# wwood/CoverM

Measured on AMD Instinct MI355X. Metric: aligned reads/s through coverm contig (mean trimmed_mean covered_fraction variance), higher is better.
Workload: dtype i32 depth / u64 sums / f32 estimators

## Files before the change

### coverm_amd/csrc/covermhip.hip

```cpp
#include "pileup_kernels.hip.h"
#include "prep_lean.hip.h"
#include "genome_kernels.hip.h"
#include "sep_kernels.hip.h"
#include "ingest_kernels.hip.h"
#include "group_kernels.hip.h"
#include "sam_kernels.hip.h"

#include <algorithm>
#include <atomic>
#include <cstddef>
#include <chrono>
#include <cstdio>
#include <dlfcn.h>
#include <functional>
#include <sched.h>
#include <cstdlib>
#include <cstring>
#include <map>
#include <mutex>
#include <string>
#include <future>
#include <thread>
#include <vector>

// ... 911 lines not shown
    if (s) s->merged_valid = false;
    cov_summary local;
    cov_status st = finish_store(s, stats, (s && s->spill.active && !summary) ? &local : summary);
    if (st == COV_OK && s->spill.active) st = merge_spilled(s, stats, summary ? summary : &local);
    return st;
}

cov_status cov_finish_genomes(cov_session *s, cov_summary *summary) {
    covr::Range rr("cov_finish_genomes");
    if (!s) return COV_ERR_INVALID_ARG;
    s->merged_valid = false;
    if (s->spill.active) { s->err = "cov_finish_genomes: part of the sample's contigs left the bounded record store: cov_finish, and aggregate on the host"; return COV_ERR_STATE; }
    s->lean_finish = true;
    const cov_status st = finish_store(s, nullptr, summary);
    s->lean_finish = false;
    return st;
}

static cov_status finish_once(cov_session *s, cov_contig_stats *stats, cov_summary *summary, bool &again) {
    again = false;
    if (!s || (!stats && s->n_targets && !s->lean_finish)) return COV_ERR_INVALID_ARG;
    const bool lean = s->lean_finish;
    s->depth_all_valid = false;
    HIPCHK(hipSetDevice(s->cfg.device));
    timing_events(s);
    hipStream_t st = s->stream;
    const u32 nT = s->n_targets;
    const u32 R = (u32)s->store.n_records;
    const bool want_hist = s->cfg.want & COV_WANT_HIST, want_id = s->cfg.want & COV_WANT_IDENTITY;
    for (int k = 0; k < COV_K_COUNT; k++) { s->k_launches[k] = 0; s->k_ms[k] = 0.f; }
    bool compacted = false;
    s->est_valid = false; s->gen_valid = false;
    s->ev_fresh = -1;

    HIPCHK(s->d_runs.reserve(std::max<size_t>(1, R), st));
    const uint64_t ncig_all = s->adopted ? s->adopted_ncig : s->store.n_cigar;
    const bool long_cigars = R && ncig_all / R >= 16;
    const int prep_kernel = s->prep_kernel;
    const int prep_passes = long_cigars ? 1 : 2 * PREP_PASSES, prep_b = 1;
    const u32 prep_chunk = (u32)(256 * prep_b * prep_passes);
    const u32 prep_grid = (R + prep_chunk - 1) / prep_chunk;
    HIPCHK(s->d_part.reserve((size_t)prep_grid + 2, st));
    if (want_id) {
        if (!(s->cfg.want & COV_WANT_IDENTITY_PRIMARY_ONLY)) HIPCHK(s->d_ident.reserve(std::max<size_t>(1, R), st));
        if (!(s->cfg.want & COV_WANT_IDENTITY_NONSUPP_ONLY)) HIPCHK(s->d_identp.reserve(std::max<size_t>(1, R), st));
        HIPCHK(s->d_idch.reserve((size_t)R / ID_CH + 2, st));
    }
    if (want_hist) HIPCHK(s->d_arena.reserve((size_t)R + nT + 1, st));

    TileIdx ti{};
    ti.tile_first = s->d_tile_first.p; ti.tcnt = s->d_tcnt.p; ti.fov = s->d_fov.p; ti.shift = s->tile_shift; ti.n_tiles = s->n_tiles;
    CxIdx cx{};
    {
        const uint64_t ncig_now = s->adopted ? s->adopted_ncig : s->store.n_cigar;
        HIPCHK(s->d_cx_list.reserve((size_t)(ncig_now / CX_MIN_OPS) + 64, st));
        cx.list = s->d_cx_list.p; cx.list_cap = (u32)std::min<uint64_t>(ncig_now / CX_MIN_OPS + 64, 0xffffffffull);
        cx.cnt = s->d_cx_cnt.p; cx.cur = s->d_cx_cur.p; cx.cscan = s->d_cx_scan.p; cx.ctop = s->d_cx_top.p;
        cx.runs = s->d_cx_runs.p; cx.runs_cap = s->d_cx_runs.cap;
    }
    const Records r = records_of(s);
    const uint8_t *mask = s->have_mask ? s->d_mask.p : nullptr;
    FilterCfg f{};
    f.include_improper_pairs = s->cfg.include_improper_pairs; f.include_supplementary = s->cfg.include_supplementary;
    f.include_secondary = s->cfg.include_secondary; f.filter_single = s->cfg.filter_single;
    f.min_mapq = s->cfg.min_mapq; f.min_aligned_length = s->cfg.min_aligned_length;
    f.min_percent_identity = s->cfg.min_percent_identity; f.min_aligned_percent = s->cfg.min_aligned_percent;
    double *idp = (want_id && !(s->cfg.want & COV_WANT_IDENTITY_NONSUPP_ONLY)) ? s->d_identp.p : nullptr;
    double *idn = (want_id && !(s->cfg.want & COV_WANT_IDENTITY_PRIMARY_ONLY)) ? s->d_ident.p : nullptr;
    HIPCHK(s->d_prep_args.reserve(1, st));
    HIPCHK(s->d_gen_list.reserve((size_t)R / 64 + 2, st));
    PrepArgs pa{};
    {
        PrepHot &ph = pa.hot;
        ph.tid = r.tid; ph.pos = r.pos; ph.flag = r.flag; ph.nmk = r.nm_kind; ph.nm = r.nm; ph.coff = r.cigar_off; ph.cigar = r.cigar; ph.mapq = r.mapq; ph.lseq = r.l_seq;
        ph.runs = s->d_runs.p; ph.tcnt = ti.tcnt; ph.fov = ti.fov; ph.identp = idp; ph.identn = idn;
        ph.n = r.n; ph.cigar_end = r.cigar_end; ph.n_targets = nT; ph.shift = ti.shift; ph.steps = (u32)prep_chunk / 256u;
        ph.gate_mask = 0x4u | (f.include_secondary ? 0u : 0x100u) | (f.include_supplementary ? 0u : 0x800u) | (f.include_improper_pairs ? 0u : 0x2u);
        ph.p1_mask = 0x4u | (f.include_secondary ? 0u : 0x100u) | (f.include_supplementary ? 0u : 0x800u);
        ph.min_mapq = f.min_mapq; ph.min_aligned_length = f.min_aligned_length; ph.min_percent_identity = f.min_percent_identity; ph.min_aligned_percent = f.min_aligned_percent;
        PrepCold &pc = pa.cold;
        pc.ctg = s->d_ctg.p; pc.g = s->d_glob.p; pc.part = s->d_part.p; pc.cx_list = cx.list; pc.mask = mask; pc.tlen = s->d_tlen.p; pc.tile_first = s->d_tile_first.p;
        pc.cx_list_cap = cx.list_cap; pc.gen_list = s->d_gen_list.p;
    }
    hipLaunchKernelGGL(k_init, dim3((std::max(std::max(nT, COUNTER_SLOTS * 8), s->n_tiles) + 255) / 256), dim3(256), 0, st, s->d_ctg.p,
                       nT, s->d_glob.p, ti, cx, s->d_prep_args.p, pa);
    HIPCHK(hipGetLastError());

    if (R) {
        time_begin(s, COV_K_PREP);
        const u32 n_steps = (R + 63u) / 64u;
        const bool gen_all = prep_kernel != 7 && (uint64_t)R < (uint64_t)nT * 128u;
        s->last_gen_all = gen_all;
        const u32 gen_grid = gen_all ? std::min<u32>((u32)s->n_cus * 64u, (n_steps + 3u) / 4u) : std::min<u32>((u32)s->n_cus * 8u, (n_steps + 3u) / 4u);
#define COV_LAUNCH_PREP(ID, FI, MA)                                                                                                       \
        do {                                                                                                                              \
            if (prep_kernel == 7)                                                                                                         \
                hipLaunchKernelGGL((k_prep7s<ID, FI, MA>), dim3(prep_grid), dim3(256), 0, st, r, s->d_tlen.p, nT, mask, f, s->d_ctg.p,   \
                                   s->d_glob.p, s->d_runs.p, idp, idn, s->d_part.p, ti, prep_passes, prep_b, cx.list, cx.list_cap);      \
            else if (gen_all)                                                                                                             \
                hipLaunchKernelGGL((k_prep_generic<ID, FI, MA>), dim3(gen_grid), dim3(256), 0, st, (const PrepArgs *)s->d_prep_args.p, n_steps); \
            else {                                                                                                                        \
                hipLaunchKernelGGL((k_prep_lean<ID, FI, MA>), dim3(prep_grid), dim3(256), 0, st, pa.hot, (const PrepArgs *)s->d_prep_args.p); \
                hipLaunchKernelGGL((k_prep_generic<ID, FI, MA>), dim3(gen_grid), dim3(256), 0, st, (const PrepArgs *)s->d_prep_args.p, 0u); \
            }                                                                                                                             \
        } while (0)
        {
            const int key = (want_id ? 4 : 0) | (s->cfg.filter_single ? 2 : 0) | (mask != nullptr ? 1 : 0);
            switch (key) {
            case 0: COV_LAUNCH_PREP(false, false, false); break;
            case 1: COV_LAUNCH_PREP(false, false, true); break;
            case 2: COV_LAUNCH_PREP(false, true, false); break;
            case 3: COV_LAUNCH_PREP(false, true, true); break;
            case 4: COV_LAUNCH_PREP(true, false, false); break;
            case 5: COV_LAUNCH_PREP(true, false, true); break;
            case 6: COV_LAUNCH_PREP(true, true, false); break;
            default: COV_LAUNCH_PREP(true, true, true); break;
            }
        }
#undef COV_LAUNCH_PREP
        if (nT) {
            const u32 n_red = gen_all ? 0u : (nT + 3u) / 4u, cx_grid0 = (u32)s->n_cus * 8u;
            hipLaunchKernelGGL(k_post_prep, dim3(n_red + cx_grid0), dim3(256), 0, st, r, s->d_tlen.p, s->d_glob.p, cx, ti, s->d_ctg.p, nT, (const PrepPartial *)s->d_part.p,
                               prep_grid, prep_chunk, n_red);
        }
        time_end(s, COV_K_PREP);
        HIPCHK(hipGetLastError());
        if (want_id && nT) {
            if (!s->side) {
                (void)ingest_prep_wait(s);
                if (s->ing_aux && !s->ing_active) s->side = s->ing_aux;
                else { HIPCHK(hipStreamCreateWithFlags(&s->side, hipStreamNonBlocking)); s->side_owned = true; }
            }
            HIPCHK(hipEventRecord(s->ev_prep_done, st));
            HIPCHK(hipStreamWaitEvent(s->side, s->ev_prep_done, 0));
            (void)hipEventRecord(s->ev[COV_K_IDENTITY][0], s->side);
            if (s->id_mode) {
                const u32 nch = (R + ID_CH - 1) / ID_CH;
                hipLaunchKernelGGL(k_id_approx, dim3(nch), dim3(256), 0, s->side, idp, idn, R, s->d_idch.p);
                hipLaunchKernelGGL(k_id_predict, dim3(nT), dim3(64), 0, s->side, s->d_ctg.p, nT, idp, idn, s->d_idch.p);
                hipLaunchKernelGGL(k_id_exact, dim3(nch), dim3(256), 0, s->side, idp, idn, R, s->d_idch.p);
                hipLaunchKernelGGL(k_id_combine, dim3(nT), dim3(64), 0, s->side, s->d_ctg.p, nT, idp, idn, r.tid, s->d_idch.p);
            } else
                hipLaunchKernelGGL(k_identity, dim3(nT), dim3(64), 0, s->side, s->d_ctg.p, nT, idp, idn, r.tid);
            (void)hipEventRecord(s->ev[COV_K_IDENTITY][1], s->side);
            s->k_launches[COV_K_IDENTITY]++;
            HIPCHK(hipGetLastError());
            HIPCHK(hipEventRecord(s->ev_side_done, s->side));
            s->ev_fresh = -1;
        }
    }
    if (R && s->n_tiles) {
        time_begin(s, COV_K_RANGES);
        const u32 n_blocks = (s->n_tiles + 1023u) / 1024u;
        const u32 cx_grid = (u32)s->n_cus * 8u;
        ScanPair sp{};
        sp.cnt[0] = s->d_tcnt.p; sp.scan[0] = s->d_tscan.p; sp.top[0] = s->d_ttop.p; sp.total[0] = nullptr;
        sp.cnt[1] = s->d_cx_cnt.p; sp.scan[1] = s->d_cx_scan.p; sp.top[1] = s->d_cx_top.p; sp.total[1] = &s->d_glob.p->cx_total;
        hipLaunchKernelGGL(k_tile_scan1, dim3(2u * n_blocks), dim3(1024), 0, st, sp, s->n_tiles, n_blocks);
        hipLaunchKernelGGL(k_tile_scan2, dim3(2), dim3(1024), 0, st, sp, n_blocks);
        hipLaunchKernelGGL((k_cx_expand<true>), dim3(cx_grid), dim3(256), 0, st, r, s->d_tlen.p, s->d_glob.p, cx, ti);
        u32 *slow_list = s->use_fast ? s->d_slow_list.p : nullptr;
        if (want_hist)
            hipLaunchKernelGGL((k_ranges<true>), dim3((s->n_tiles + 255) / 256), dim3(256), 0, st, s->d_tile_contig.p,
                               s->d_tile_start.p, s->n_tiles, s->d_tlen.p, mask, s->d_ctg.p, s->d_desc.p, ti, s->d_tscan.p,
                               s->d_ttop.p, cx, s->d_glob.p, slow_list);
        else
            hipLaunchKernelGGL((k_ranges<false>), dim3((s->n_tiles + 255) / 256), dim3(256), 0, st, s->d_tile_contig.p,
                               s->d_tile_start.p, s->n_tiles, s->d_tlen.p, mask, s->d_ctg.p, s->d_desc.p, ti, s->d_tscan.p,
                               s->d_ttop.p, cx, s->d_glob.p, slow_list);
        time_end(s, COV_K_RANGES);
        HIPCHK(hipGetLastError());
        if (want_hist) {
            time_begin(s, COV_K_HIST);
            const u32 hb = (nT + 1023u) / 1024u;
            HIPCHK(s->d_hist_top.reserve(hb, st));
            hipLaunchKernelGGL((k_hist_sum<0>), dim3(hb), dim3(1024), 0, st, (const DevContig *)s->d_ctg.p, nT, s->d_tlen.p, mask, (u64)s->cfg.contig_end_exclusion, s->d_hist_top.p);
            hipLaunchKernelGGL((k_hist_off<0>), dim3(hb), dim3(1024), 0, st, s->d_ctg.p, nT, s->d_tlen.p, mask, (u64)s->cfg.contig_end_exclusion, (const u64 *)s->d_hist_top.p, s->d_glob.p);
            hipLaunchKernelGGL(k_zero_u32, dim3(2048), dim3(256), 0, st, s->d_arena.p, &s->d_glob.p->hist_cap_total);
            time_end(s, COV_K_HIST);
            HIPCHK(hipGetLastError());
        }
        PileupArgs a = pileup_args(s);
        time_begin(s, COV_K_PILEUP);
        if (want_hist) launch_any_pileup<true, false>(s, a, s->n_tiles);
        else launch_any_pileup<false, false>(s, a, s->n_tiles);
        time_end(s, COV_K_PILEUP);
        HIPCHK(hipGetLastError());
        if (want_hist) {
            compacted = s->est.n == 0 || s->hist_fetch_seen;
            s->hist_prefetched = 0;
            if (compacted) {
                HIPCHK(s->d_chist.reserve((size_t)R + nT + 1, st));
                time_begin(s, COV_K_HIST_COMPACT);
                const u32 hb = (nT + 1023u) / 1024u;
                hipLaunchKernelGGL((k_hist_sum<1>), dim3(hb), dim3(1024), 0, st, (const DevContig *)s->d_ctg.p, nT, s->d_tlen.p, mask, (u64)s->cfg.contig_end_exclusion, s->d_hist_top.p);
                hipLaunchKernelGGL((k_hist_off<1>), dim3(hb), dim3(1024), 0, st, s->d_ctg.p, nT, s->d_tlen.p, mask, (u64)s->cfg.contig_end_exclusion, (const u64 *)s->d_hist_top.p, s->d_glob.p);
                hipLaunchKernelGGL(k_hist_compact, dim3((nT + 3u) / 4u), dim3(256), 0, st, s->d_ctg.p, nT, s->d_tlen.p, (u64)s->cfg.contig_end_exclusion, s->d_arena.p, s->d_chist.p);
                time_end(s, COV_K_HIST_COMPACT);
                HIPCHK(hipGetLastError());
                const u64 guess = s->hist_fetch_seen ? std::min<u64>({s->last_chist_total + s->last_chist_total / 16, (u64)R + nT + 1, (u64)(64u << 20) / 8}) : 0;
                if (guess) {
                    if (guess > s->h_chist_cap) {
                        if (s->h_chist) (void)hipHostFree(s->h_chist);
                        s->h_chist = nullptr; s->h_chist_cap = 0;
                        HIPCHK(hipHostMalloc((void **)&s->h_chist, (size_t)guess * 8, hipHostMallocDefault));
                        s->h_chist_cap = guess;
                    }
                    HIPCHK(hipMemcpyAsync(s->h_chist, s->d_chist.p, (size_t)guess * 8, hipMemcpyDeviceToHost, st));
                    s->hist_prefetched = guess;
                }
            }
            s->hist_fetch_seen = false;
        }
    }
    const size_t block = result_block_bytes(nT), nf = (s->have_mask || s->have_runs) ? 0 : (size_t)nT * s->est.n;
    {
        result_host_take(s);
        const size_t need = lean ? sizeof(DevGlobal) + sizeof(DevContig) : result_host_bytes(s, nT);
        if (need > s->h_res_cap) {
            if (s->h_res) (void)hipHostFree(s->h_res);
            s->h_res = nullptr; s->h_res_cap = 0;
            const size_t cap = need < ((size_t)64 << 20) ? need + need / 2 : need;
            HIPCHK(hipHostMalloc((void **)&s->h_res, cap, hipHostMallocDefault));
            s->h_res_cap = cap;
        }
        s->h_ctg = (DevContig *)(s->h_res + sizeof(DevGlobal));
        s->h_estf = reinterpret_cast<float *>(s->h_res + block);
    }
    if (want_id && R && nT) { HIPCHK(hipStreamWaitEvent(st, s->ev_side_done, 0)); s->ev_fresh = -1; }
    if (nf) {
        time_begin(s, COV_K_ESTIMATE);
        if (s->est_lanes < 0 ? nT >= 65536u : s->est_lanes == 1)
            hipLaunchKernelGGL(k_estimate_lanes, dim3((nT + 255) / 256), dim3(256), 0, st, (const DevContig *)s->d_ctg.p, nT, (const u32 *)s->d_tlen.p, (u64)s->cfg.contig_end_exclusion,
                               (const u32 *)s->d_arena.p, s->est, reinterpret_cast<float *>(s->d_res.p + block));
        else
            hipLaunchKernelGGL(k_estimate, dim3((nT + 3) / 4), dim3(256), 0, st, (const DevContig *)s->d_ctg.p, nT, (const u32 *)s->d_tlen.p, (u64)s->cfg.contig_end_exclusion,
                               (const u32 *)s->d_arena.p, s->est, reinterpret_cast<float *>(s->d_res.p + block));
        time_end(s, COV_K_ESTIMATE);
        HIPCHK(hipGetLastError());
    }
    const bool runs = s->have_runs && s->est.n != 0 && !s->spill.active && !s->in_spill;
    const bool genomes = runs || (s->have_genomes && s->est.n != 0 && !s->spill.active && !s->in_spill);
    if (lean && !genomes) { s->err = "cov_finish_genomes: cov_set_genomes or cov_set_genome_runs, and cov_set_estimators, first, and no spill of the bounded record store (cov_finish then)"; return COV_ERR_STATE; }
    u32 sep_counts[SEP_N_COUNTS] = {0, 0, 0, 0};
    if (runs) {
        const u32 nb = (std::max(nT, 1u) + SEP_TILE - 1u) / SEP_TILE, eb = (s->sep_ent_cap + SEP_TILE - 1u) / SEP_TILE, cap = s->sep_ent_cap;
        time_begin(s, COV_K_SEP);
        hipLaunchKernelGGL(k_sep_obs_top, dim3(nb), dim3(SEP_TILE), 0, st, (const DevContig *)s->d_ctg.p, nT, s->d_stop_last1.p, s->d_stop_first.p);
        hipLaunchKernelGGL(k_sep_flags, dim3(nb), dim3(SEP_TILE), 0, st, (const DevContig *)s->d_ctg.p, nT, (const int32_t *)s->d_sgid.p, (const u32 *)s->d_sblk.p,
                           (const u32 *)s->d_stop_last1.p, (const u32 *)s->d_stop_first.p, s->d_scode.p, s->d_stop_cnt.p);
        hipLaunchKernelGGL(k_sep_compact, dim3(nb), dim3(SEP_TILE), 0, st, nT, (const int32_t *)s->d_sgid.p, (const u32 *)s->d_sblk.p, (const uint8_t *)s->d_scode.p,
                           (const u64 *)s->d_stop_cnt.p, s->d_gtids.p, s->d_sent_pos.p, s->d_sent.p, cap, s->d_scounts.p, s->d_glob.p);
        hipLaunchKernelGGL(k_sep_rows, dim3((std::max(nT, 1u) + 255u) / 256u), dim3(256), 0, st, (const u32 *)s->d_scounts.p, (const u32 *)s->d_sent_pos.p, s->d_grow.p, cap);
        hipLaunchKernelGGL(k_sep_seg_sum, dim3(eb), dim3(SEP_TILE), 0, st, (const u32 *)s->d_scounts.p, (const u32 *)s->d_grow.p, s->d_stop_seg.p);
        hipLaunchKernelGGL(k_sep_seg_write, dim3(eb), dim3(SEP_TILE), 0, st, s->d_scounts.p, (const u32 *)s->d_grow.p, (const u64 *)s->d_stop_seg.p, s->d_gseg_genome.p,
                           s->d_gseg_start.p, s->sep_seg_cap);
        time_end(s, COV_K_SEP);
        HIPCHK(hipGetLastError());
        uint8_t *hc = s->h_gout + s->h_gout_cap - 16;
        HIPCHK(hipMemcpyAsync(hc, s->d_scounts.p, SEP_N_COUNTS * sizeof(u32), hipMemcpyDeviceToHost, st));
        HIPCHK(hipStreamSynchronize(st));
        memcpy(sep_counts, hc, sizeof sep_counts);
        s->ev_fresh = -1;
        s->n_genomes = sep_counts[SEP_N_ENTRIES]; s->n_gseg = sep_counts[SEP_N_SEG];
    }
    if (genomes && s->n_genomes != 0) {
        const u32 nG = s->n_genomes, n_seg = s->n_gseg, sep = runs ? 1u : 0u;
        GenomeTable gt{s->d_grow.p, s->d_gtids.p, s->d_gseg_genome.p, s->d_gseg_start.p, nG, n_seg};
        const u64 excl = s->cfg.contig_end_exclusion;
        const u64 ghist_cap = (u64)R + nT + 1;
        if (want_hist) HIPCHK(s->d_ghist.reserve((size_t)ghist_cap, st));
        time_begin(s, COV_K_GENOME);
        hipLaunchKernelGGL(k_genome_init, dim3((nG + 255u) / 256u), dim3(256), 0, st, s->d_genomes.p, nG);
        if (n_seg) hipLaunchKernelGGL(k_genome_reduce, dim3((n_seg + 3u) / 4u), dim3(256), 0, st, (const DevContig *)s->d_ctg.p, (const u32 *)s->d_tlen.p, excl, gt, s->d_genomes.p, sep);
        if (want_id && !(s->cfg.want & (runs ? COV_WANT_IDENTITY_NONSUPP_ONLY : COV_WANT_IDENTITY_PRIMARY_ONLY)))
            hipLaunchKernelGGL(k_genome_identity, dim3(nG), dim3(64), 0, st, (const DevContig *)s->d_ctg.p, gt, s->d_genomes.p, sep);
        if (want_hist) {
            const u32 gb = (nG + 1023u) / 1024u;
            u64 *total = s->d_ghist_top.p + gb;
            hipLaunchKernelGGL(k_genome_hist_sum, dim3(gb), dim3(1024), 0, st, (const DevGenome *)s->d_genomes.p, nG, s->d_ghist_top.p);
            hipLaunchKernelGGL(k_genome_hist_off, dim3(gb), dim3(1024), 0, st, s->d_genomes.p, nG, (const u64 *)s->d_ghist_top.p, total, ghist_cap, s->d_glob.p);
            hipLaunchKernelGGL(k_zero_u64, dim3(1024), dim3(256), 0, st, s->d_ghist.p, (const u64 *)total, ghist_cap);
            if (n_seg && R && s->n_tiles)
                hipLaunchKernelGGL(k_genome_hist_merge, dim3((n_seg + 3u) / 4u), dim3(256), 0, st, (const DevContig *)s->d_ctg.p, (const u32 *)s->d_tlen.p, excl,
                                   (const u32 *)s->d_arena.p, gt, (const DevGenome *)s->d_genomes.p, s->d_ghist.p, ghist_cap);
        }
        DevGenomeStats *gstats = reinterpret_cast<DevGenomeStats *>(s->d_gout.p);
        float *gest = reinterpret_cast<float *>(s->d_gout.p + (size_t)nG * sizeof(DevGenomeStats));
        if (nG >= 65536u)
            hipLaunchKernelGGL(k_genome_estimate_lanes, dim3((nG + 255u) / 256u), dim3(256), 0, st, (const DevGenome *)s->d_genomes.p, nG, (const u64 *)s->d_ghist.p, s->est, gest, gstats);
        else
            hipLaunchKernelGGL(k_genome_estimate, dim3((nG + 3u) / 4u), dim3(256), 0, st, (const DevGenome *)s->d_genomes.p, nG, (const u64 *)s->d_ghist.p, s->est, gest, gstats);
        time_end(s, COV_K_GENOME);
        HIPCHK(hipGetLastError());
        HIPCHK(hipMemcpyAsync(s->h_gout, s->d_gout.p, (size_t)nG * (sizeof(DevGenomeStats) + s->est.n * sizeof(float)), hipMemcpyDeviceToHost, st));
        if (runs) HIPCHK(hipMemcpyAsync(s->h_gout + (size_t)nG * (sizeof(DevGenomeStats) + s->est.n * sizeof(float)), s->d_sent.p, (size_t)nG * sizeof(SepEntry), hipMemcpyDeviceToHost, st));
    }
    if (lean) {
        const u32 ob = (nT + 1023u) / 1024u;
        HIPCHK(s->d_order.reserve((size_t)ob + 2, st));
        hipLaunchKernelGGL(k_order_max, dim3(std::max(ob, 1u)), dim3(1024), 0, st, (const DevContig *)s->d_ctg.p, nT, s->d_order.p);
        hipLaunchKernelGGL(k_order_check, dim3(std::max(ob, 1u)), dim3(1024), 0, st, (const DevContig *)s->d_ctg.p, nT, s->d_order.p);
        HIPCHK(hipGetLastError());
        HIPCHK(hipMemcpyAsync(s->h_res, s->d_res.p, sizeof(DevGlobal), hipMemcpyDeviceToHost, st));
        HIPCHK(hipMemcpyAsync(s->h_res + sizeof(DevGlobal), s->d_order.p, 8, hipMemcpyDeviceToHost, st));
    } else
    HIPCHK(hipMemcpyAsync(s->h_res, s->d_res.p, sizeof(DevGlobal) + (size_t)nT * sizeof(DevContig) + (nf ? (block - sizeof(DevGlobal) - (size_t)nT * sizeof(DevContig)) + nf * sizeof(float) : 0),
                          hipMemcpyDeviceToHost, st));
    {
        const auto t_spin = std::chrono::steady_clock::now();
        for (;;) {
            const hipError_t q = hipStreamQuery(st);
            if (q == hipSuccess) break;
            if (q != hipErrorNotReady) { (void)hipGetLastError(); break; }
            (void)hipGetLastError();
            if (std::chrono::steady_clock::now() - t_spin > std::chrono::milliseconds(4)) break;
            __builtin_ia32_pause();
        }
    }
    HIPCHK(hipStreamSynchronize(st));
    memcpy(&s->h_glob, s->h_res, sizeof(DevGlobal));
    if (s->h_glob.cx_total > s->d_cx_runs.cap) {
// ... 1469 lines not shown
```

### coverm_amd/csrc/pileup_kernels.hip.h

```cpp
#pragma once
#include <hip/hip_runtime.h>
#include <stdint.h>

namespace covk {

typedef unsigned long long u64;
typedef unsigned int u32;

constexpr u32 F_POS_UNSORTED = 1u;
constexpr u32 RW_SINGLE = 0u, RW_DOUBLE = 1u, RW_COMPLEX = 2u, RW_BUCKET = 3u;
constexpr u32 FAST_MAX_CAND = 8191u;
constexpr u32 TILE_F_GENERIC = 1u, TILE_F_SLOW = 2u;
constexpr u32 CX_MIN_OPS = 16;

struct DevContig {
    u64 n_primary, n_pass, n_nonsupp, sum_nm, sum_indel;
    double id_primary, id_nonsupp;
    u64 sum_d, sum_d2, cov_win, cov_full, proc_win;
    u64 hist_off;
    u32 first_rec, last_rec;
    u32 rec_start, rec_end;
    u32 n_groups;
    u32 max_span;
    u32 flags;
// ... 533 lines not shown
                const u32 key = tv ? t0[k] + tl : 0xffffffffu;
                const u32 pk = (u32)__builtin_amdgcn_update_dpp((int)0xffffffffu, (int)key, 0x138, 0xf, 0xf, false);
                const bool lead = tv && (lane == 0 || key != pk);
                const u64 bm = __ballot(lead) | ~__ballot(tv);
                if (lead) {
                    const u64 rest = (bm >> lane) >> 1;
                    const u32 follow = rest ? (u32)__builtin_ctzll(rest) : (u32)(63 - lane);
                    atomicAdd(&ti.tcnt[key], 1u + follow);
                }
                const u32 e = span > L - pc ? L : pc + span;
                const u32 te = (tv && span > 0u) ? (e - 1u) >> ti.shift : 0u;
                const bool cross = tv && masked_in && n_runs > 0u && span > 0u && te > tl && !is_bucket;
                const u64 cm = __ballot(cross);
                if (cm != 0) {
                    const int fl0 = __ffsll((long long)cm) - 1;
                    const u32 tgt = key + 1u, tgt0 = __builtin_amdgcn_readlane(tgt, fl0);
                    if (__all(!cross || (te == tl + 1u && tgt == tgt0))) { if (lane == fl0) atomicMin(&ti.fov[tgt0], i); }
                    else if (cross) for (u32 t2 = tl + 1u; t2 <= te; t2++) atomicMin(&ti.fov[t0[k] + t2], i);
                }
            }

            const bool cnt = considered && tid_ok;
            const u64 m = __ballot(cnt);
            g_cons += (u32)__popcll(m);
            if (m != 0) {
                const int ftid = __shfl(tid, __ffsll((long long)m) - 1);
                const bool uni = __all(!cnt || tid == ftid);
                if (uni) {
                    if (ftid != cur) { if (cur >= 0) flushed_early = true; prep_flush(ctg, cur, acc); cur = ftid; }
                    acc.prim += (u32)__popcll(__ballot(cnt && !supp && !sec));
                    acc.pass += (u32)__popcll(m);
                    acc.nons += (u32)__popcll(__ballot(cnt && !supp));
                    if (cnt) {
                        acc.first = min(acc.first, i); acc.last = max(acc.last, i);
                        if (masked_in) { acc.nm += nmv; acc.indel += indel; acc.span = max(acc.span, span); }
                    }
                } else {
                    prep_flush(ctg, cur, acc); cur = -1; flushed_early = true;
                    if (cnt) {
                        DevContig *C = &ctg[tid];
                        if (!supp && !sec) atomicAdd(&C->n_primary, 1ull);
                        atomicAdd(&C->n_pass, 1ull);
                        if (!supp) atomicAdd(&C->n_nonsupp, 1ull);
                        if (masked_in) {
                            if (nmv) atomicAdd(&C->sum_nm, nmv);
                            if (indel) atomicAdd(&C->sum_indel, indel);
                            atomicMax(&C->max_span, span);
                        }
                        atomicMin(&C->first_rec, i);
                        atomicMax(&C->last_rec, i);
                    }
                }
            }
        }
    }
    {
        PrepPartial pw;
        pw.tid = flushed_early ? -2 : cur;
        pw.prim = acc.prim; pw.pass = acc.pass; pw.nons = acc.nons;
        pw.span = wave_max_u32(acc.span); pw.first = wave_min_u32(acc.first); pw.last = wave_max_u32(acc.last);
        pw.nm = wave_sum_u64(acc.nm); pw.indel = wave_sum_u64(acc.indel); pw.pad = 0;
        if (lane == 0) wpart[w] = pw;
    }
    if (lane == 0) { blk_cnt[0][w] = g_prim; blk_cnt[1][w] = g_cons; }
    __syncthreads();
    bool uniform_wg = true;
    {
        int t0 = -1;
        for (int k = 0; k < 4; k++) {
            const int t = wpart[k].tid;
            if (t == -2) uniform_wg = false;
            else if (t >= 0) { if (t0 < 0) t0 = t; else if (t != t0) uniform_wg = false; }
        }
        if (threadIdx.x == 0) {
            PrepPartial o; o.tid = -1; o.prim = o.pass = o.nons = o.span = 0; o.first = 0xffffffffu; o.last = 0; o.pad = 0; o.nm = o.indel = 0;
            if (uniform_wg && t0 >= 0) {
                o.tid = t0;
                for (int k = 0; k < 4; k++) {
                    const PrepPartial &q = wpart[k];
                    if (q.tid < 0) continue;
                    o.prim += q.prim; o.pass += q.pass; o.nons += q.nons; o.span = max(o.span, q.span);
                    o.first = min(o.first, q.first); o.last = max(o.last, q.last); o.nm += q.nm; o.indel += q.indel;
                }
            }
            part[blockIdx.x] = o;
        }
    }
    if (!uniform_wg) prep_flush(ctg, cur, acc);
    if (threadIdx.x == 0) {
        const u32 p = blk_cnt[0][0] + blk_cnt[0][1] + blk_cnt[0][2] + blk_cnt[0][3];
        const u32 c = blk_cnt[1][0] + blk_cnt[1][1] + blk_cnt[1][2] + blk_cnt[1][3];
        const u32 slot = (blockIdx.x % COUNTER_SLOTS) * 8u;
        if (p) atomicAdd(&g->prim_slots[slot], (u64)p);
        if (c) atomicAdd(&g->cons_slots[slot], (u64)c);
    }
}

#define COV_PREP_KERNEL(NAME, ATTR, PF, PB)                                                                                                           \
    template <bool WANT_IDENTITY, bool FILTER, bool MASKED>                                                                                      \
    __global__ __launch_bounds__(256) ATTR void NAME(Records r, const u32 *__restrict__ tlen, u32 n_targets, const uint8_t *__restrict__ mask,   \
                                                     FilterCfg f, DevContig *ctg, DevGlobal *g, uint2 *__restrict__ runs,                        \
                                                     double *__restrict__ identp, double *__restrict__ identn, PrepPartial *__restrict__ part,   \
                                                     TileIdx ti, int passes, int b_active, u32 *__restrict__ cx_list, u32 cx_list_cap) {         \
        prep_body<WANT_IDENTITY, FILTER, MASKED, PF, PB>(r, tlen, n_targets, mask, f, ctg, g, runs, identp, identn, part, ti, passes, b_active, cx_list, \
                                                 cx_list_cap);                                                                                   \
    }
COV_PREP_KERNEL(k_prep7s, __attribute__((amdgpu_waves_per_eu(7, 7))), true, 1)
#undef COV_PREP_KERNEL

__device__ __forceinline__ void prep_reduce_body(u32 c, DevContig *ctg, u32 n_targets, const PrepPartial *__restrict__ part, u32 n_parts, u32 chunk_recs) {
    if (c >= n_targets) return;
    DevContig *C = &ctg[c];
    const u32 rs = C->rec_start, re = C->rec_end;
    if (rs >= re) return;
    const u32 b0 = rs / chunk_recs, b1 = min((re - 1) / chunk_recs, n_parts - 1);
    u32 prim = 0, pass = 0, nons = 0, span = 0, first = 0xffffffffu, last = 0;
    u64 nm = 0, indel = 0;
    for (u32 b = b0 + (threadIdx.x & 63); b <= b1; b += 64) {
        const PrepPartial q = part[b];
        if (q.tid != (int)c) continue;
        prim += q.prim; pass += q.pass; nons += q.nons; span = max(span, q.span);
        first = min(first, q.first); last = max(last, q.last); nm += q.nm; indel += q.indel;
    }
    prim = wave_sum_u32(prim); pass = wave_sum_u32(pass); nons = wave_sum_u32(nons); span = wave_max_u32(span);
    first = wave_min_u32(first); last = wave_max_u32(last); nm = wave_sum_u64(nm); indel = wave_sum_u64(indel);
    if ((threadIdx.x & 63) == 0 && pass) {
        C->n_primary += prim; C->n_pass += pass; C->n_nonsupp += nons; C->sum_nm += nm; C->sum_indel += indel;
        C->max_span = max(C->max_span, span); C->first_rec = min(C->first_rec, first); C->last_rec = max(C->last_rec, last);
    }
}

__device__ __forceinline__ u32 lower_bound_pos(const int32_t *__restrict__ pos, u32 lo, u32 hi, long long key) {
    while (lo < hi) {
        const u32 mid = lo + ((hi - lo) >> 1);
        if ((long long)pos[mid] < key) lo = mid + 1; else hi = mid;
    }
    return lo;
}

struct ScanPair { const u32 *cnt[2]; u32 *scan[2]; u32 *top[2]; u64 *total[2]; };
__global__ __launch_bounds__(1024) void k_tile_scan1(ScanPair sp, u32 n_tiles, u32 n_blocks) {
    __shared__ u32 wtot[16];
    const u32 which = blockIdx.x >= n_blocks ? 1u : 0u, blk = blockIdx.x - which * n_blocks;
    const u32 *__restrict__ tcnt = sp.cnt[which];
    const u32 t = blk * 1024u + threadIdx.x;
    const int lane = lane_id(), w = threadIdx.x >> 6;
    const u32 v = t < n_tiles ? tcnt[t] : 0u;
    const u32 inc = (u32)wave_incl_scan((int)v);
    if (lane == 63) wtot[w] = inc;
    __syncthreads();
    u32 wbase = 0, tot = 0;
    for (int k = 0; k < 16; k++) { const u32 x = wtot[k]; if (k < w) wbase += x; tot += x; }
    if (t < n_tiles) sp.scan[which][t] = wbase + inc - v;
    if (threadIdx.x == 0) sp.top[which][blk] = tot;
}

__global__ __launch_bounds__(1024) void k_tile_scan2(ScanPair sp, u32 n_blocks) {
    __shared__ u32 wtot[16];
    __shared__ u32 carry_s;
    u32 *ttop = sp.top[blockIdx.x];
    u64 *total = sp.total[blockIdx.x];
    if (threadIdx.x == 0) carry_s = 0;
    __syncthreads();
    const int lane = lane_id(), w = threadIdx.x >> 6;
    for (u32 base = 0; base < n_blocks; base += 1024u) {
        const u32 b = base + threadIdx.x;
        const u32 v = b < n_blocks ? ttop[b] : 0u;
        const u32 inc = (u32)wave_incl_scan((int)v);
        if (lane == 63) wtot[w] = inc;
        __syncthreads();
        u32 wbase = 0, tot = 0;
        for (int k = 0; k < 16; k++) { const u32 x = wtot[k]; if (k < w) wbase += x; tot += x; }
        const u32 carry = carry_s;
        if (b < n_blocks) ttop[b] = carry + wbase + inc - v;
        __syncthreads();
        if (threadIdx.x == 0) carry_s = carry + tot;
        __syncthreads();
    }
    if (total != nullptr && threadIdx.x == 0) *total = carry_s;
}

template <bool FILL>
__device__ __forceinline__ void cx_expand_body(const Records &r, const u32 *__restrict__ tlen, DevGlobal *g, const CxIdx &cx, const TileIdx &ti, u32 wave, u32 n_waves) {
    const int lane = lane_id();
    const u32 n = min(g->n_cx, cx.list_cap);
    if (FILL && g->cx_total > cx.runs_cap) return;
    const u64 lt = lane == 0 ? 0ull : (~0ull >> (64 - lane));
    for (u32 j = wave; j < n; j += n_waves) {
        const u32 i = cx.list[j];
        const int tid = r.tid[i];
        const u32 co0 = r.cigar_off[i], nops = r.cigar_off[i + 1] - co0;
        const u32 L = tlen[tid], t0 = ti.tile_first[tid];
        long long cur0 = r.pos[i];
        u32 wd_next = (u32)lane < nops ? r.cigar[co0 + (u32)lane] : 4u;
        for (u32 base = 0; base < nops; base += 64) {
            const u32 wd = wd_next;
            const u32 idn = base + 64u + (u32)lane;
            wd_next = idn < nops ? r.cigar[co0 + idn] : 4u;
            const u32 len = wd >> 4, bit = 1u << (wd & 15u);
            const u32 fr = (bit & 0x18du) ? len : 0u;
            const u32 incl = (u32)wave_incl_scan((int)fr), excl = incl - fr;
            const long long sj = cur0 + (long long)excl;
            const bool m = (bit & 0x181u) != 0u && len > 0u && sj >= 0 && sj < (long long)L;
            const u32 sv = (u32)sj, ev = sv + len;
            const u32 ts = sv >> ti.shift, te = m ? (min(ev, L) - 1u) >> ti.shift : 0u;
            for (u32 k = 0; __any(m && ts + k <= te); k++) {
                const bool v = m && ts + k <= te;
                const u32 key = t0 + ts + k;
                u32 slot = 0;
                for (u64 todo = __ballot(v); todo != 0;) {
                    const int l = __ffsll((long long)todo) - 1;
                    const u32 k0 = __builtin_amdgcn_readlane(key, l);
                    const u64 grp = __ballot(v && key == k0);
                    u32 b = 0;
                    if (lane == l) b = atomicAdd(FILL ? &cx.cur[k0] : &cx.cnt[k0], (u32)__popcll(grp));
                    if (FILL) {
                        b = __builtin_amdgcn_readlane(b, l);
                        if (v && key == k0) slot = b + (u32)__popcll(grp & lt);
                    }
                    todo &= ~grp;
                }
                if (FILL && v) cx.runs[(u64)cx.cscan[key] + cx.ctop[key >> 10] + slot] = make_uint2(sv, ev);
            }
            cur0 += (long long)__builtin_amdgcn_readlane(incl, 63);
        }
    }
}

template <bool FILL>
__global__ __launch_bounds__(256) void k_cx_expand(Records r, const u32 *__restrict__ tlen, DevGlobal *g, CxIdx cx, TileIdx ti) {
    cx_expand_body<FILL>(r, tlen, g, cx, ti, blockIdx.x * 4u + (threadIdx.x >> 6), gridDim.x * 4u);
}

__global__ __launch_bounds__(256) void k_post_prep(Records r, const u32 *__restrict__ tlen, DevGlobal *g, CxIdx cx, TileIdx ti, DevContig *ctg, u32 n_targets,
                                                   const PrepPartial *__restrict__ part, u32 n_parts, u32 chunk_recs, u32 n_red) {
    if (blockIdx.x < n_red) prep_reduce_body(blockIdx.x * 4u + (threadIdx.x >> 6), ctg, n_targets, part, n_parts, chunk_recs);
    else cx_expand_body<false>(r, tlen, g, cx, ti, (blockIdx.x - n_red) * 4u + (threadIdx.x >> 6), (gridDim.x - n_red) * 4u);
}

template <bool WANT_HIST>
__global__ __launch_bounds__(256) void k_ranges(const u32 *__restrict__ tile_contig, const u32 *__restrict__ tile_start,
                                                u32 n_tiles, const u32 *__restrict__ tlen, const uint8_t *__restrict__ mask,
                                                DevContig *ctg, uint4 *__restrict__ desc, TileIdx ti,
                                                const u32 *__restrict__ tscan, const u32 *__restrict__ ttop, CxIdx cx,
                                                DevGlobal *__restrict__ g, u32 *__restrict__ slow_list) {
    const u32 t = blockIdx.x * blockDim.x + threadIdx.x;
    if (t >= n_tiles) return;
    const u32 c = tile_contig[t];
    DevContig *C = &ctg[c];
    uint4 out = make_uint4(0u, 0u, tlen[c], 0u);
    u32 cxn = 0, cxo = 0;
    if (C->n_pass != 0 && (mask == nullptr || mask[c])) {
        const u32 rs = C->rec_start, re = C->rec_end;
        cxn = g->cx_total <= cx.runs_cap ? cx.cnt[t] : 0u;
        cxo = cx.cscan[t] + cx.ctop[t >> 10];
        if (C->n_groups != 1u) out.w = 1u;
        if (C->n_groups != 1u || (C->flags & F_POS_UNSORTED)) {
            out.x = rs; out.y = re;
        } else {
            const u32 tf = ti.tile_first[c];
            const u32 before = (tscan[t] + ttop[t >> 10]) - (tscan[tf] + ttop[tf >> 10]);
            const u32 f = rs + before;
            out.y = min(f + ti.tcnt[t], re);
            out.x = max(min(f, ti.fov[t]), rs);
            out.x = min(out.x, out.y);
        }
    }
    if (out.x < out.y || cxn) {
        if (out.w || out.y - out.x + cxn > FAST_MAX_CAND) {
            out.w |= TILE_F_SLOW;
            if (slow_list != nullptr) slow_list[atomicAdd(&g->n_slow, 1u)] = t;
        }
    }
    if (WANT_HIST) {
        const u32 npass = (u32)min(C->n_pass, (u64)0xffffffffu);
        const u32 cap = min(out.y - out.x + cxn, npass);
        if (__all(c == (u32)__builtin_amdgcn_readfirstlane((int)c))) {
            const u32 m = wave_max_u32(cap);
            if (lane_id() == 0 && m) atomicMax(&C->hist_cap, m);
        } else if (cap) atomicMax(&C->hist_cap, cap);
    }
    desc[2 * t] = out;
    desc[2 * t + 1] = make_uint4(c, tile_start[t], cxo, cxn);
}

template <int MODE>
__device__ __forceinline__ u64 hist_bins_of(const DevContig *C, u32 c, const u32 *__restrict__ tlen, const uint8_t *__restrict__ mask, u64 excl) {
    const bool live = C->n_pass != 0 && (mask == nullptr || mask[c]);
    if (MODE == 0) return live ? (u64)C->hist_cap + 1 : 0;
    return (live && 2 * excl < (u64)tlen[c]) ? (u64)C->max_d + 1 : 0;
}
__device__ __forceinline__ u64 block_incl_scan_u64(u64 v, u64 *wtot, u64 &total) {
    const int lane = lane_id(), w = threadIdx.x >> 6;
    u64 inc = v;
#pragma unroll
    for (int o = 1; o < 64; o <<= 1) {
        const u64 t = __shfl_up(inc, o);
        if (lane >= o) inc += t;
    }
    if (lane == 63) wtot[w] = inc;
    __syncthreads();
    u64 wbase = 0; total = 0;
    for (int k = 0; k < 16; k++) { const u64 x = wtot[k]; if (k < w) wbase += x; total += x; }
    __syncthreads();
    return wbase + inc;
}
template <int MODE>
__global__ __launch_bounds__(1024) void k_hist_sum(const DevContig *__restrict__ ctg, u32 n_targets, const u32 *__restrict__ tlen,
                                                   const uint8_t *__restrict__ mask, u64 excl, u64 *__restrict__ top) {
    __shared__ u64 wtot[16];
    const u32 c = blockIdx.x * 1024u + threadIdx.x;
    u64 total;
    (void)block_incl_scan_u64(c < n_targets ? hist_bins_of<MODE>(&ctg[c], c, tlen, mask, excl) : 0, wtot, total);
    if (threadIdx.x == 0) top[blockIdx.x] = total;
}
template <int MODE>
__global__ __launch_bounds__(1024) void k_hist_off(DevContig *ctg, u32 n_targets, const u32 *__restrict__ tlen, const uint8_t *__restrict__ mask,
                                                   u64 excl, const u64 *__restrict__ top, DevGlobal *g) {
    __shared__ u64 wtot[16];
    u64 mine = 0, base;
    for (u32 b = threadIdx.x; b < blockIdx.x; b += 1024u) mine += top[b];
    (void)block_incl_scan_u64(mine, wtot, base);
    const u32 c = blockIdx.x * 1024u + threadIdx.x;
    const u64 v = c < n_targets ? hist_bins_of<MODE>(&ctg[c], c, tlen, mask, excl) : 0;
    u64 total;
    const u64 inc = block_incl_scan_u64(v, wtot, total);
    if (c < n_targets) {
        if (MODE == 0) ctg[c].hist_off = base + inc - v;
        else { ctg[c].chist_off = base + inc - v; ctg[c].hist_len = (u32)v; }
    }
    if (blockIdx.x == gridDim.x - 1 && threadIdx.x == 0) {
        if (MODE == 0) g->hist_cap_total = base + total; else g->chist_total = base + total;
    }
}

__global__ void k_zero_u32(u32 *__restrict__ p, const u64 *__restrict__ n_ptr) {
    const u64 n = *n_ptr;
    for (u64 i = (u64)blockIdx.x * blockDim.x + threadIdx.x; i < n; i += (u64)gridDim.x * blockDim.x) p[i] = 0u;
}

__global__ __launch_bounds__(256) void k_hist_compact(const DevContig *__restrict__ ctg, u32 n_targets,
                                                      const u32 *__restrict__ tlen, u64 excl,
                                                      const u32 *__restrict__ arena, u64 *__restrict__ out) {
    const u32 c = blockIdx.x * 4u + (threadIdx.x >> 6);
    if (c >= n_targets) return;
    const DevContig *C = &ctg[c];
    const u32 n = C->hist_len;
    if (n == 0) return;
    const u64 win_len = (u64)tlen[c] - 2 * excl;
    for (u32 d = threadIdx.x & 63u; d < n; d += 64u) {
        u64 v = arena[C->hist_off + d];
        if (d == 0) v += win_len - C->proc_win;
        out[C->chist_off + d] = v;
    }
}

__global__ __launch_bounds__(64) void k_identity(DevContig *ctg, u32 n_targets, const double *__restrict__ identp,
                                                 const double *__restrict__ identn, const int32_t *__restrict__ tidv) {
    const u32 c = blockIdx.x;
    if (c >= n_targets) return;
    DevContig *C = &ctg[c];
    if (C->n_pass == 0) return;
    const u32 rs = C->rec_start, re = C->rec_end;
    const bool generic = C->n_groups != 1u;
    double accp = 0.0, accn = 0.0;
    const int lane = lane_id();
    u32 i = rs + (u32)lane;
    double xp = 0.0, xn = 0.0;
    if (i < re && (!generic || tidv[i] == (int)c)) { if (identp) xp = identp[i]; if (identn) xn = identn[i]; }
    for (u32 b = rs; b < re; b += 64) {
        const double cp = xp, cn = xn;
        i += 64;
        xp = 0.0; xn = 0.0;
        if (i < re && (!generic || tidv[i] == (int)c)) { if (identp) xp = identp[i]; if (identn) xn = identn[i]; }
#pragma unroll 16
        for (int k = 0; k < 64; k++) {
            accn += __shfl(cn, k);
            accp += __shfl(cp, k);
        }
    }
    if (lane == 0) { C->id_primary = accp; C->id_nonsupp = accn; }
}

constexpr u32 ID_CH = 1024;
struct IdChunk {
    double ap, an;
    u64 tp, tn;
    int ep, en;
    u32 flags;
    u32 pad;
};
constexpr int ID_SERIAL = -2147483647 - 1;

__device__ __forceinline__ int f64_exp(double v) { return (int)((__double_as_longlong(v) >> 52) & 0x7ff) - 1023; }

__global__ __launch_bounds__(256) void k_id_approx(const double *__restrict__ identp, const double *__restrict__ identn,
                                                   u32 n, IdChunk *__restrict__ ch) {
    __shared__ double sp[4], sn[4];
    __shared__ u32 sf[4];
    const u32 k = blockIdx.x, base = k * ID_CH;
    double ap = 0.0, an = 0.0;
    u32 fl = 0;
#pragma unroll
    for (int j = 0; j < (int)(ID_CH / 256); j++) {
        const u32 i = base + (u32)j * 256u + threadIdx.x;
        if (i < n) {
            const double xp = identp ? identp[i] : 0.0, xn = identn ? identn[i] : 0.0;
            if (!(xp >= 0.0 && xp <= 1.0)) fl |= 1u;
            if (!(xn >= 0.0 && xn <= 1.0)) fl |= 2u;
            ap += xp; an += xn;
        }
    }
#pragma unroll
    for (int o = 32; o > 0; o >>= 1) { ap += __shfl_xor(ap, o); an += __shfl_xor(an, o); fl |= __shfl_xor(fl, o); }
    const int w = threadIdx.x >> 6;
    if ((threadIdx.x & 63) == 0) { sp[w] = ap; sn[w] = an; sf[w] = fl; }
    __syncthreads();
    if (threadIdx.x == 0) {
        IdChunk c;
        c.ap = sp[0] + sp[1] + sp[2] + sp[3]; c.an = sn[0] + sn[1] + sn[2] + sn[3];
        c.tp = c.tn = 0; c.ep = c.en = ID_SERIAL; c.flags = sf[0] | sf[1] | sf[2] | sf[3]; c.pad = 0;
        ch[k] = c;
    }
}

__global__ __launch_bounds__(64) void k_id_predict(const DevContig *__restrict__ ctg, u32 n_targets,
                                                   const double *__restrict__ identp, const double *__restrict__ identn,
                                                   IdChunk *__restrict__ ch) {
    const u32 c = blockIdx.x;
    if (c >= n_targets) return;
    const DevContig *C = &ctg[c];
    if (C->n_pass == 0 || C->n_groups != 1u) return;
    const u32 rs = C->rec_start, re = C->rec_end;
    const u32 k0 = (rs + ID_CH - 1) / ID_CH, k1 = re / ID_CH;
    if (k0 >= k1) return;
    double pp = 0.0, pn = 0.0;
// ... 945 lines not shown
```

Before: 48.25 billion.

## Drop second scan pass and fuse complex-read expansion into ranges kernel

Removes the k_tile_scan2 block-prefix pass. Consumers now rebuild block offsets on the fly by summing per-block totals (wave/block reductions in k_ranges, a cached incremental sum in cx_expand), and the cx total comes from an atomicAdd in scan1. The separate k_cx_expand launch is folded into k_ranges as extra leading blocks, cutting two kernel launches and their serialization on the stream. In exchange each block does redundant prefix summation over the per-block totals, which grows with tile count, and the expansion now runs concurrently with range building. cx_total must start at zero before scan1 for the atomic accumulation to be correct.

```diff
diff --git a/coverm_amd/csrc/covermhip.hip b/coverm_amd/csrc/covermhip.hip
--- a/coverm_amd/csrc/covermhip.hip
+++ b/coverm_amd/csrc/covermhip.hip
@@ -1087,22 +1087,20 @@
     if (R && s->n_tiles) {
         time_begin(s, COV_K_RANGES);
         const u32 n_blocks = (s->n_tiles + 1023u) / 1024u;
-        const u32 cx_grid = (u32)s->n_cus * 8u;
+        const u32 n_fill = (u32)s->n_cus * 8u;
         ScanPair sp{};
         sp.cnt[0] = s->d_tcnt.p; sp.scan[0] = s->d_tscan.p; sp.top[0] = s->d_ttop.p; sp.total[0] = nullptr;
         sp.cnt[1] = s->d_cx_cnt.p; sp.scan[1] = s->d_cx_scan.p; sp.top[1] = s->d_cx_top.p; sp.total[1] = &s->d_glob.p->cx_total;
         hipLaunchKernelGGL(k_tile_scan1, dim3(2u * n_blocks), dim3(1024), 0, st, sp, s->n_tiles, n_blocks);
-        hipLaunchKernelGGL(k_tile_scan2, dim3(2), dim3(1024), 0, st, sp, n_blocks);
-        hipLaunchKernelGGL((k_cx_expand<true>), dim3(cx_grid), dim3(256), 0, st, r, s->d_tlen.p, s->d_glob.p, cx, ti);
         u32 *slow_list = s->use_fast ? s->d_slow_list.p : nullptr;
         if (want_hist)
-            hipLaunchKernelGGL((k_ranges<true>), dim3((s->n_tiles + 255) / 256), dim3(256), 0, st, s->d_tile_contig.p,
+            hipLaunchKernelGGL((k_ranges<true>), dim3(n_fill + (s->n_tiles + 255) / 256), dim3(256), 0, st, s->d_tile_contig.p,
                                s->d_tile_start.p, s->n_tiles, s->d_tlen.p, mask, s->d_ctg.p, s->d_desc.p, ti, s->d_tscan.p,
-                               s->d_ttop.p, cx, s->d_glob.p, slow_list);
+                               s->d_ttop.p, cx, s->d_glob.p, slow_list, r, n_fill);
         else
-            hipLaunchKernelGGL((k_ranges<false>), dim3((s->n_tiles + 255) / 256), dim3(256), 0, st, s->d_tile_contig.p,
+            hipLaunchKernelGGL((k_ranges<false>), dim3(n_fill + (s->n_tiles + 255) / 256), dim3(256), 0, st, s->d_tile_contig.p,
                                s->d_tile_start.p, s->n_tiles, s->d_tlen.p, mask, s->d_ctg.p, s->d_desc.p, ti, s->d_tscan.p,
-                               s->d_ttop.p, cx, s->d_glob.p, slow_list);
+                               s->d_ttop.p, cx, s->d_glob.p, slow_list, r, n_fill);
         time_end(s, COV_K_RANGES);
         HIPCHK(hipGetLastError());
         if (want_hist) {
diff --git a/coverm_amd/csrc/pileup_kernels.hip.h b/coverm_amd/csrc/pileup_kernels.hip.h
--- a/coverm_amd/csrc/pileup_kernels.hip.h
+++ b/coverm_amd/csrc/pileup_kernels.hip.h
@@ -709,32 +709,19 @@
     u32 wbase = 0, tot = 0;
     for (int k = 0; k < 16; k++) { const u32 x = wtot[k]; if (k < w) wbase += x; tot += x; }
     if (t < n_tiles) sp.scan[which][t] = wbase + inc - v;
-    if (threadIdx.x == 0) sp.top[which][blk] = tot;
-}
-
-__global__ __launch_bounds__(1024) void k_tile_scan2(ScanPair sp, u32 n_blocks) {
-    __shared__ u32 wtot[16];
-    __shared__ u32 carry_s;
-    u32 *ttop = sp.top[blockIdx.x];
-    u64 *total = sp.total[blockIdx.x];
-    if (threadIdx.x == 0) carry_s = 0;
-    __syncthreads();
-    const int lane = lane_id(), w = threadIdx.x >> 6;
-    for (u32 base = 0; base < n_blocks; base += 1024u) {
-        const u32 b = base + threadIdx.x;
-        const u32 v = b < n_blocks ? ttop[b] : 0u;
-        const u32 inc = (u32)wave_incl_scan((int)v);
-        if (lane == 63) wtot[w] = inc;
-        __syncthreads();
-        u32 wbase = 0, tot = 0;
-        for (int k = 0; k < 16; k++) { const u32 x = wtot[k]; if (k < w) wbase += x; tot += x; }
-        const u32 carry = carry_s;
-        if (b < n_blocks) ttop[b] = carry + wbase + inc - v;
-        __syncthreads();
-        if (threadIdx.x == 0) carry_s = carry + tot;
-        __syncthreads();
-    }
-    if (total != nullptr && threadIdx.x == 0) *total = carry_s;
+    if (threadIdx.x == 0) {
+        sp.top[which][blk] = tot;
+        if (sp.total[which] != nullptr && tot) atomicAdd(sp.total[which], (u64)tot);
+    }
+}
+
+__device__ __forceinline__ u32 cx_block_base(const u32 *__restrict__ top, u32 kb, u32 &ckb, u32 &cbase) {
+    if (kb == ckb) return cbase;
+    u32 lo = 0, acc = 0, part = 0;
+    if (kb > ckb) { lo = ckb; acc = cbase; }
+    for (u32 b = lo + (u32)lane_id(); b < kb; b += 64u) part += top[b];
+    ckb = kb; cbase = acc + wave_sum_u32_dpp(part);
+    return cbase;
 }
 
 template <bool FILL>
@@ -743,6 +730,7 @@
     const u32 n = min(g->n_cx, cx.list_cap);
     if (FILL && g->cx_total > cx.runs_cap) return;
     const u64 lt = lane == 0 ? 0ull : (~0ull >> (64 - lane));
+    u32 ckb = 0, cbase = 0;
     for (u32 j = wave; j < n; j += n_waves) {
         const u32 i = cx.list[j];
         const int tid = r.tid[i];
@@ -777,16 +765,21 @@
                     }
                     todo &= ~grp;
                 }
-                if (FILL && v) cx.runs[(u64)cx.cscan[key] + cx.ctop[key >> 10] + slot] = make_uint2(sv, ev);
+                if (FILL) {
+                    u32 base = 0;
+                    for (u64 todo = __ballot(v); todo != 0;) {
+                        const int l = __ffsll((long long)todo) - 1;
+                        const u32 kb = __builtin_amdgcn_readlane(key >> 10, l);
+                        const u32 b = cx_block_base(cx.ctop, kb, ckb, cbase);
+                        if ((key >> 10) == kb) base = b;
+                        todo &= ~__ballot(v && (key >> 10) == kb);
+                    }
+                    if (v) cx.runs[(u64)cx.cscan[key] + base + slot] = make_uint2(sv, ev);
+                }
             }
             cur0 += (long long)__builtin_amdgcn_readlane(incl, 63);
         }
     }
-}
-
-template <bool FILL>
-__global__ __launch_bounds__(256) void k_cx_expand(Records r, const u32 *__restrict__ tlen, DevGlobal *g, CxIdx cx, TileIdx ti) {
-    cx_expand_body<FILL>(r, tlen, g, cx, ti, blockIdx.x * 4u + (threadIdx.x >> 6), gridDim.x * 4u);
 }
 
 __global__ __launch_bounds__(256) void k_post_prep(Records r, const u32 *__restrict__ tlen, DevGlobal *g, CxIdx cx, TileIdx ti, DevContig *ctg, u32 n_targets,
@@ -800,23 +793,40 @@
                                                 u32 n_tiles, const u32 *__restrict__ tlen, const uint8_t *__restrict__ mask,
                                                 DevContig *ctg, uint4 *__restrict__ desc, TileIdx ti,
                                                 const u32 *__restrict__ tscan, const u32 *__restrict__ ttop, CxIdx cx,
-                                                DevGlobal *__restrict__ g, u32 *__restrict__ slow_list) {
-    const u32 t = blockIdx.x * blockDim.x + threadIdx.x;
-    if (t >= n_tiles) return;
-    const u32 c = tile_contig[t];
+                                                DevGlobal *__restrict__ g, u32 *__restrict__ slow_list, Records r, u32 n_fill) {
+    __shared__ u32 red[8];
+    if (blockIdx.x < n_fill) {
+        cx_expand_body<true>(r, tlen, g, cx, ti, blockIdx.x * 4u + (threadIdx.x >> 6), n_fill * 4u);
+        return;
+    }
+    const u32 t0 = (blockIdx.x - n_fill) * 256u;
+    const bool in = t0 + threadIdx.x < n_tiles;
+    const u32 t = in ? t0 + threadIdx.x : n_tiles - 1u;
+    const u32 c = tile_contig[t], blk = t0 >> 10;
+    const u32 blk_f0 = ti.tile_first[tile_contig[t0]] >> 10, n_cx = g->n_cx;
+    u32 rec_top = 0, cx_top = 0;
+    if (blk_f0 < blk || (n_cx != 0u && blk != 0u)) {
+        u32 a = 0, b = 0;
+        for (u32 k = blk_f0 + threadIdx.x; k < blk; k += 256u) a += ttop[k];
+        if (n_cx != 0u) for (u32 k = threadIdx.x; k < blk; k += 256u) b += cx.ctop[k];
+        a = wave_sum_u32_dpp(a); b = wave_sum_u32_dpp(b);
+        if (lane_id() == 0) { red[threadIdx.x >> 6] = a; red[4 + (threadIdx.x >> 6)] = b; }
+        __syncthreads();
+        rec_top = red[0] + red[1] + red[2] + red[3]; cx_top = red[4] + red[5] + red[6] + red[7];
+    }
     DevContig *C = &ctg[c];
     uint4 out = make_uint4(0u, 0u, tlen[c], 0u);
     u32 cxn = 0, cxo = 0;
     if (C->n_pass != 0 && (mask == nullptr || mask[c])) {
         const u32 rs = C->rec_start, re = C->rec_end;
         cxn = g->cx_total <= cx.runs_cap ? cx.cnt[t] : 0u;
-        cxo = cx.cscan[t] + cx.ctop[t >> 10];
+        cxo = cx.cscan[t] + cx_top;
         if (C->n_groups != 1u) out.w = 1u;
         if (C->n_groups != 1u || (C->flags & F_POS_UNSORTED)) {
             out.x = rs; out.y = re;
         } else {
             const u32 tf = ti.tile_first[c];
-            const u32 before = (tscan[t] + ttop[t >> 10]) - (tscan[tf] + ttop[tf >> 10]);
+            const u32 before = (tscan[t] - tscan[tf]) + ((tf >> 10) < blk ? rec_top : 0u);
             const u32 f = rs + before;
             out.y = min(f + ti.tcnt[t], re);
             out.x = max(min(f, ti.fov[t]), rs);
@@ -826,7 +836,7 @@
     if (out.x < out.y || cxn) {
         if (out.w || out.y - out.x + cxn > FAST_MAX_CAND) {
             out.w |= TILE_F_SLOW;
-            if (slow_list != nullptr) slow_list[atomicAdd(&g->n_slow, 1u)] = t;
+            if (in && slow_list != nullptr) slow_list[atomicAdd(&g->n_slow, 1u)] = t;
         }
     }
     if (WANT_HIST) {
@@ -837,8 +847,10 @@
             if (lane_id() == 0 && m) atomicMax(&C->hist_cap, m);
         } else if (cap) atomicMax(&C->hist_cap, cap);
     }
-    desc[2 * t] = out;
-    desc[2 * t + 1] = make_uint4(c, tile_start[t], cxo, cxn);
+    if (in) {
+        desc[2 * t] = out;
+        desc[2 * t + 1] = make_uint4(c, tile_start[t], cxo, cxn);
+    }
 }
 
 template <int MODE>
```

After: 48.51 billion, median of 5. Within noise of the previous version (+0.5%).
